# Kiripiro/leaffliction

Measured on AMD Instinct MI355X. Metric: 224x224 images/sec train, higher is better.
Workload: dtype f32; 1 GPU; leaf_cnn base train step (configs[1]: img 224, batch 256/GPU, fp32, 8 classes, AdamW+clipnorm+EMA, in-model augmentation); per_gpu_batch=256, global_batch=256, img_size=224, parallelism=dp1

## Files before the change

include/leafhip.h:

```cpp
#ifndef LEAFHIP_H
#define LEAFHIP_H

#include <stddef.h>
#include <stdint.h>

#ifdef __cplusplus
extern "C" {
#endif

#define LF_OK 0
#define LF_ERR_INVALID (-1)
#define LF_ERR_LAUNCH (-2)
#define LF_ERR_WORKSPACE (-3)

#define LF_VERSION 100

typedef void* lf_stream_t;

int lf_version(void);
const char* lf_last_error(void);

int lf_copy_rows(void* dst, size_t dst_pitch, const void* src, size_t src_pitch, size_t width, size_t rows, int to_host,
                 lf_stream_t stream);

// ... 122 lines not shown
                               const int32_t* ohw, const int64_t* out_off, int n, int h, int w,
                               int max_out_pixels, int fill, lf_stream_t stream);

int lf_resample_u8(const uint8_t* in, uint8_t* tmp, uint8_t* out, int n, int h, int w, int oh,
                   int ow, const int32_t* xbounds, const int32_t* xk, int kx,
                   const int32_t* ybounds, const int32_t* yk, int ky, int per_image_coeffs,
                   lf_stream_t stream);

int lf_resample_tile_u8(const uint8_t* in, uint8_t* out, int n, int h, int w, int oh, int ow,
                        const int32_t* xbounds, const int32_t* xk, int kx, const int32_t* ybounds,
                        const int32_t* yk, int ky, int per_image_coeffs, lf_stream_t stream);


int lf_conv2d_f32(const float* x, const float* w, float* y, int n, int cin, int h, int wd, int cout,
                  int ksize, const float* in_scale, const float* in_shift, int in_relu,
                  int accumulate, lf_stream_t stream);

size_t lf_conv2d_bf16_weight_elems(int cin, int cout, int ksize);
int lf_conv2d_bf16_prep_weights(const float* w_iko, uint16_t* wprep, int cin, int cout, int ksize,
                                lf_stream_t stream);
int lf_conv2d_bf16_f32(const float* x, const uint16_t* wprep, float* y, int n, int cin, int h, int wd,
                       int cout, int ksize, const float* in_scale, const float* in_shift, int in_relu,
                       lf_stream_t stream);

int lf_conv2d_bf16_act(const void* x, int x_bf16, const uint16_t* wprep, void* y, int y_bf16, int n,
                       int cin, int h, int wd, int cout, int ksize, const float* in_scale,
                       const float* in_shift, int in_relu, const float* out_scale,
                       const float* out_shift, int out_relu, lf_stream_t stream);
size_t lf_conv2d_bf16_act_mean_workspace(int n, int cin, int h, int wd, int cout, int ksize, int x_bf16);
int lf_conv2d_bf16_act_mean(const void* x, int x_bf16, const uint16_t* wprep, uint16_t* y, int n, int cin,
                            int h, int wd, int cout, int ksize, const float* in_scale,
// ... 32 lines not shown
int lf_cast_bf16_f32(const uint16_t* in, float* out, size_t count, lf_stream_t stream);

int lf_conv2d_variant(int h, int wd, int cout, int ksize);
int lf_conv2d_wgrad_variant(int n, int cin, int h, int wd, int cout, int ksize);

int lf_conv2d_plan(int n, int cin, int h, int wd, int cout, int ksize, int* out);
int lf_conv2d_wgrad_plan(int n, int cin, int h, int wd, int cout, int ksize, int* out);
int lf_conv2d_bf16_plan(int n, int cin, int h, int w, int cout, int ksize, int x_bf16, int y_bf16, int entry,
                        int accumulate, int mask, int* out);
int lf_conv2d_wgrad_bf16_plan(int n, int cin, int h, int w, int cout, int ksize, int* out);

long long lf_conv2d_stats_tiles(int n, int cin, int h, int w, int cout, int ksize);
int lf_conv2d_stats_f32(const float* x, const float* w, float* y, int n, int cin, int h, int wd,
                        int cout, int ksize, const float* in_scale, const float* in_shift,
                        int in_relu, const float* pivot, float* tile_part, size_t tile_part_bytes,
                        lf_stream_t stream);

int lf_conv2d_bnbwd_f32(const float* x, const float* w, float* y, int n, int cin, int h, int wd,
                        int cout, int ksize, int accumulate, const float* mask_y,
                        const float* mask_scale, const float* mask_shift, int mask_relu,
                        float* tile_part, size_t tile_part_bytes, lf_stream_t stream);

int lf_conv2d_dgrad_weights_f32(const float* w, float* wt, int cin, int ksize, int cout,
                                lf_stream_t stream);

size_t lf_conv2d_wgrad_workspace(int n, int cin, int h, int wd, int cout, int ksize);
int lf_conv2d_wgrad_f32(const float* x, const float* dy, int n, int cin, int h, int wd, int cout,
                        int ksize, const float* in_scale, const float* in_shift, int in_relu,
                        void* workspace, size_t ws_bytes, lf_stream_t stream);
int lf_conv2d_wgrad_reduce_f32(void* workspace, float* dw, int n, int cin, int h, int wd,
                               int cout, int ksize, float beta, lf_stream_t stream);
int lf_conv2d_wgrad_bn_supported(int n, int cin, int h, int w, int cout, int ksize);
int lf_conv2d_wgrad_bn_f32(const float* x, const float* g, const float* bn_y,
                           const float* alpha_nc, const float* add_nc, const float* coef,
                           int bn_relu, float* dy_out, int n, int cin, int h, int w, int cout,
                           int ksize, const float* in_scale, const float* in_shift, int in_relu,
                           void* workspace, size_t ws_bytes, lf_stream_t stream);

int lf_input_stage_f32(const uint8_t* in, float* out, int n, int h, int w, const float* aug4,
// ... 78 lines not shown
```

leaffliction_amd/_lib.py:

```python
from __future__ import annotations

import ctypes as C
import os
from pathlib import Path

_LIB = None

LIB_PATH = Path(__file__).resolve().parent / "libleafhip.so"

c_void_p, c_int, c_size_t, c_u64, c_float, c_double = (
    C.c_void_p, C.c_int, C.c_size_t, C.c_uint64, C.c_float, C.c_double)
P = c_void_p

SIGNATURES = {
    "lf_version": [],
    "lf_last_error": [],
    "lf_pack_hwc_u8_to_nchw_f32": [P, P, c_int, c_int, c_int, P, P, P],
    "lf_hist_u8": [P, P, c_int, c_int, c_int, P],
    "lf_autocontrast_lut": [P, P, P, c_int, P],
    "lf_lut_apply_u8": [P, P, P, c_int, c_int, c_int, P],
    "lf_gather_rows_u8": [P, P, P, c_int, c_size_t, P],
    "lf_flip_u8": [P, P, P, c_int, c_int, c_int, P],
    "lf_noise_wrap_add_u8": [P, P, P, c_size_t, P],
    "lf_add_wrap_u8": [P, P, P, c_size_t, P],
# ... 27 lines not shown
    "lf_inclusive_mask_u8": [P, P, c_int, c_int, c_int, c_int, c_int, P, P, c_size_t, P],
    "lf_make_mask_workspace": [c_int, c_int, c_int, c_int, c_int],
    "lf_make_mask_u8": [P, P, P, P, P, c_int, c_int, c_int, c_int, c_int, c_int, c_double, P, c_int, P, P,
                        c_size_t, P],
    "lf_brown_spots_workspace": [c_int, c_int, c_int],
    "lf_brown_spots_u8": [P, P, P, P, P, c_int, c_int, c_int, P, P, c_size_t, P],
    "lf_roi_u8": [P, P, P, c_int, P, P, P, P, c_int, c_int, c_int, c_int, c_int, P],
    "lf_blur_saliency_workspace": [c_int, c_int, c_int],
    "lf_blur_saliency_u8": [P, P, P, c_int, c_int, c_int, c_int, c_int, c_int, c_int, c_int, P, P, P,
                            c_size_t, P],
    "lf_warp_bicubic_u8": [P, P, P, c_int, c_int, c_int, c_int, P],
    "lf_affine_nearest_fixed_u8": [P, P, P, P, P, c_int, c_int, c_int, c_int, c_int, P],
    "lf_resample_tile_u8": [P, P, c_int, c_int, c_int, c_int, c_int, P, P, c_int, P, P, c_int, c_int, P],
    "lf_resample_u8": [P, P, P, c_int, c_int, c_int, c_int, c_int, P, P, c_int, P, P, c_int,
                       c_int, P],
    "lf_conv2d_f32": [P, P, P, c_int, c_int, c_int, c_int, c_int, c_int, P, P, c_int, c_int, P],
    "lf_conv2d_bf16_weight_elems": [c_int, c_int, c_int],
    "lf_conv2d_bf16_prep_weights": [P, P, c_int, c_int, c_int, P],
    "lf_conv2d_bf16_f32": [P, P, P, c_int, c_int, c_int, c_int, c_int, c_int, P, P, c_int, P],
    "lf_conv2d_bf16_act": [P, c_int, P, P, c_int, c_int, c_int, c_int, c_int, c_int, c_int, P, P, c_int,
                           P, P, c_int, P],
    "lf_conv2d_bf16_act_mean_workspace": [c_int, c_int, c_int, c_int, c_int, c_int, c_int],
    "lf_conv2d_bf16_act_mean": [P, c_int, P, P, c_int, c_int, c_int, c_int, c_int, c_int, P, P, c_int, P, P, c_int, P, P,
                                c_size_t, P],
    "lf_conv2d_bf16_stats_tiles": [c_int, c_int, c_int, c_int, c_int, c_int, c_int],
    "lf_conv2d_bf16_train": [P, c_int, P, P, c_int, c_int, c_int, c_int, c_int, c_int, P, P, c_int, c_int, P,
                             c_size_t, P, P, P, P, c_int, P],
    "lf_conv2d_wgrad_bf16_workspace": [c_int, c_int, c_int, c_int, c_int, c_int],
    "lf_conv2d_wgrad_bf16": [P, P, P, P, P, P, c_int, P, P, c_int, c_int, c_int, c_int, c_int, c_int, P, P,
                             c_int, P, c_size_t, P],
    "lf_gap_stats_bf16": [P, P, P, c_int, c_int, c_int, P, P, c_int, P],
    "lf_block_tail_fwd_train_bf16": [P, P, P, P, P, P, P, c_int, P, P, P, c_int, c_int, c_int, c_int, P],
    "lf_block_tail_bwd_bf16": [P, P, P, P, P, P, P, P, P, P, P, c_int, c_int, c_int, c_int, P],
    "lf_bcast_planes_bf16": [P, P, c_int, c_int, c_float, P],
    "lf_cast_f32_bf16": [P, P, c_size_t, P],
    "lf_cast_bf16_f32": [P, P, c_size_t, P],
    "lf_conv2d_variant": [c_int, c_int, c_int, c_int],
    "lf_conv2d_wgrad_variant": [c_int, c_int, c_int, c_int, c_int, c_int],
    "lf_conv2d_plan": [c_int, c_int, c_int, c_int, c_int, c_int, P],
    "lf_conv2d_wgrad_plan": [c_int, c_int, c_int, c_int, c_int, c_int, P],
    "lf_conv2d_bf16_plan": [c_int, c_int, c_int, c_int, c_int, c_int, c_int, c_int, c_int, c_int, c_int, P],
    "lf_conv2d_wgrad_bf16_plan": [c_int, c_int, c_int, c_int, c_int, c_int, P],
    "lf_conv2d_stats_tiles": [c_int, c_int, c_int, c_int, c_int, c_int],
    "lf_conv2d_stats_f32": [P, P, P, c_int, c_int, c_int, c_int, c_int, c_int, P, P, c_int, P, P, c_size_t, P],
    "lf_conv2d_bnbwd_f32": [P, P, P, c_int, c_int, c_int, c_int, c_int, c_int, c_int, P, P, P, c_int, P,
                            c_size_t, P],
    "lf_conv2d_dgrad_weights_f32": [P, P, c_int, c_int, c_int, P],
    "lf_conv2d_wgrad_workspace": [c_int, c_int, c_int, c_int, c_int, c_int],
    "lf_conv2d_wgrad_f32": [P, P, c_int, c_int, c_int, c_int, c_int, c_int, P, P, c_int, P,
                            c_size_t, P],
    "lf_conv2d_wgrad_bn_supported": [c_int, c_int, c_int, c_int, c_int, c_int],
    "lf_conv2d_wgrad_bn_f32": [P, P, P, P, P, P, c_int, P, c_int, c_int, c_int, c_int, c_int, c_int, P, P,
                               c_int, P, c_size_t, P],
    "lf_conv2d_wgrad_reduce_f32": [P, P, c_int, c_int, c_int, c_int, c_int, c_int, c_float, P],
    "lf_input_stage_f32": [P, P, c_int, c_int, c_int, P, P, P, P, P],
    "lf_scale_shift_act_f32": [P, P, c_int, c_int, c_int, P, P, c_int, P],
    "lf_bn_workspace": [c_int],
    "lf_bn_train_stats_f32": [P, c_int, c_int, c_int, P, P, P, P, c_float, c_float, P, P, P, P,
                              P, c_size_t, P],
    "lf_bn_train_stats_tiles_f32": [P, C.c_longlong, c_int, c_int, c_int, P, P, P, P, c_float, c_float, P, P, P, P, P, c_size_t, P],
    "lf_bn_bwd_sums_f32": [P, P, P, P, P, P, P, P, c_int, P, P, P, P, P, P, c_int, c_int, c_int, P,
                           c_size_t, P],
# ... 63 lines not shown
```

leaffliction_amd/csrc/lf_conv.hip:

```cpp
#include <type_traits>

#include "lf_common.h"

namespace {

typedef float f32x16 __attribute__((ext_vector_type(16)));
typedef float f32x4 __attribute__((ext_vector_type(4)));

constexpr int kThreads = 256;

__device__ __forceinline__ float pro_apply(float v, float sc, float sh, int relu) {
    v = fmaf(v, sc, sh);
    return relu ? fmaxf(v, 0.f) : v;
}

typedef float lf_f4 __attribute__((ext_vector_type(4)));
constexpr unsigned kBufOob = 0xffffffffu;
__device__ __forceinline__ __amdgpu_buffer_rsrc_t buf_rsrc(const float* base, unsigned bytes) {
    return __builtin_amdgcn_make_buffer_rsrc(const_cast<float*>(base), 0, bytes, 0x00020000);
}
__device__ __forceinline__ float4 buf_load4(__amdgpu_buffer_rsrc_t r, unsigned off) {
    const lf_f4 v = __builtin_bit_cast(lf_f4, __builtin_amdgcn_raw_buffer_load_b128(r, off, 0, 0));
    return make_float4(v.x, v.y, v.z, v.w);
}
__device__ __forceinline__ float buf_load1(__amdgpu_buffer_rsrc_t r, unsigned off) {
    return __builtin_bit_cast(float, __builtin_amdgcn_raw_buffer_load_b32(r, off, 0, 0));
}

struct ConvArgs {
    const float* x;
    const float* w;
    float* y;
    const float* in_scale;
    const float* in_shift;
    int n, cin, cout, h, wd;
    int tiles_x, tiles_y;
    int in_relu;
    int accumulate;
    int vec_ok;
    int stack;
    float* stat_part;
    const float* stat_pivot;
    long long stat_tiles;
    const float* stat_mask_y;
    const float* mask_scale;
    const float* mask_shift;
// ... 523 lines not shown
                    d[r * 4 + 0] = lo.x;
                    d[r * 4 + 1] = lo.y;
                    d[r * 4 + 2] = hi.x;
                    d[r * 4 + 3] = hi.y;
                }
                wino_input(d, v);
#pragma unroll
                for (int m = 0; m < MB; ++m)
#pragma unroll
                    for (int q = 0; q < 16; ++q)
                        wacc[m][nb][q] = __builtin_amdgcn_mfma_f32_16x16x4f32(u[m][q], v[q], wacc[m][nb][q], 0, 0, 0);
            }
        }
    };

    static_assert(kKC * CT <= kThreads, "one (channel, cout) filter per thread");
    const int ukc = tid / CT, uco = tid - ukc * CT;
    const bool u_on = tid < kKC * CT;
    const unsigned ugo = (u_on && co0 + uco < p.cout) ? 4u * ((unsigned)ukc * 9u * (unsigned)p.cout + (unsigned)(co0 + uco)) : kBufOob;
    float wr[9];
    auto load_u = [&](int c0) {
        const __amdgpu_buffer_rsrc_t rw =
            buf_rsrc(p.w + (size_t)c0 * 9 * p.cout, 4u * (unsigned)(min(kKC, p.cin - c0) * 9) * (unsigned)p.cout);
#pragma unroll
        for (int tap = 0; tap < 9; ++tap)
            wr[tap] = buf_load1(rw, ugo == kBufOob ? kBufOob : ugo + 4u * (unsigned)tap * (unsigned)p.cout);
    };
    auto store_u = [&]() {
        if (u_on) {
            float u[16];
            wino_filter(wr, u);
            float4* dst = reinterpret_cast<float4*>(lw + (ukc * CT + uco) * kUP);
#pragma unroll
            for (int q4 = 0; q4 < 4; ++q4) dst[q4] = make_float4(u[4 * q4], u[4 * q4 + 1], u[4 * q4 + 2], u[4 * q4 + 3]);
        }
    };

    const int nchunks = (p.cin + kKC - 1) / kKC;
    const bool vec = p.vec_ok && (t.tx0 + TW <= p.wd);

    if (vec) {
        constexpr bool kPrefetchW = NB == 1;
        Patch patch(p, t, lsc, tid);
        auto store_chunk = [&](int c0) {
            if (!kPrefetchW) load_u(c0);
            patch.store(p, lp, lsc, c0, tid);
            store_u();
        };
        patch.load(p, xin, 0);
        if (kPrefetchW) load_u(0);
        for (int ch = 0; ch < nchunks; ++ch) {
            __syncthreads();
            store_chunk(ch * kKC);
            __syncthreads();
            if (ch + 1 < nchunks) {
                patch.load(p, xin, (ch + 1) * kKC);
                if (kPrefetchW) load_u((ch + 1) * kKC);
            }
            compute_chunk();
        }
    } else {
        for (int ch = 0; ch < nchunks; ++ch) {
            const int c0 = ch * kKC;
            __syncthreads();
            Patch::stage_scalar(p, lp, xin, t.tx0, t.ty0, c0, tid);
            load_u(c0);
            store_u();
            __syncthreads();
            compute_chunk();
        }
    }

    float* yout = p.y + (size_t)t.n * p.cout * hw;
// ... 923 lines not shown
        float* o = dst + (size_t)g * count + i;
        *o = (final_pass && beta != 0.f) ? fmaf(beta, *o, s) : s;
    }
}

__global__ __launch_bounds__(kThreads) void weight_dgrad_kernel(const float* __restrict__ w,
                                                                float* __restrict__ wt, int cin,
                                                                int taps, int cout) {
    const int total = cin * taps * cout;
    for (int i = blockIdx.x * kThreads + threadIdx.x; i < total; i += gridDim.x * kThreads) {
        const int ci = i % cin, t = (i / cin) % taps, co = i / (cin * taps);
        wt[i] = w[((size_t)ci * taps + (taps - 1 - t)) * cout + co];
    }
}

struct FwdVariant {
    int tw, th, ct;
};
constexpr FwdVariant kFwdVariants[] = {{32, 8, 32}, {32, 8, 64}, {16, 16, 32}, {16, 16, 64},
                                       {28, 8, 128}, {32, 8, 128}, {56, 8, 64}};
constexpr int kNumFwd = sizeof(kFwdVariants) / sizeof(kFwdVariants[0]);

inline long long padded_work(const FwdVariant& v, int h, int w, int cout) {
    const long long tx = (w + v.tw - 1) / v.tw, ty = (h + v.th - 1) / v.th,
                    tc = (cout + v.ct - 1) / v.ct;
    return tx * v.tw * ty * v.th * tc * v.ct;
}

inline bool fwd_small_cin(int taps, int variant, int cin) { return taps == 9 && variant == 0 && cin <= 4; }

// ... 174 lines not shown
    return LF_OK;
}

int lf_conv2d_wgrad_plan(int n, int cin, int h, int wd, int cout, int ksize, int* out) {
    LF_REQUIRE(out, "lf_conv2d_wgrad_plan: null out");
    LF_REQUIRE(n > 0 && cin > 0 && cout > 0 && h > 0 && wd > 0 && (ksize == 1 || ksize == 3),
               "lf_conv2d_wgrad_plan: bad dims");
    const WgPlan pl = plan_wgrad(n, cin, cout, h, wd, ksize);
    out[0] = pl.variant;
    out[1] = pl.items_per_split < 3 ? pl.items_per_split : 3;
    out[2] = lf::slab_stages(pl.splits);
    out[3] = lf_conv2d_wgrad_bn_supported(n, cin, h, wd, cout, ksize);
    return LF_OK;
}

static int conv2d_launch(const char* who, const float* x, const float* w, float* y, int n, int cin,
                         int h, int wd, int cout, int ksize, const float* in_scale,
                         const float* in_shift, int in_relu, int accumulate, float* stat_part,
                         const float* stat_pivot, const float* stat_mask_y, const float* mask_scale,
                         const float* mask_shift, int mask_relu, lf_stream_t stream) {
    LF_REQUIRE(x && w && y, "%s: null buffer", who);
    LF_REQUIRE(n > 0 && cin > 0 && cout > 0 && h > 0 && wd > 0,
               "%s: bad dims n=%d cin=%d cout=%d h=%d w=%d", who, n, cin, cout, h, wd);
    LF_REQUIRE(ksize == 3 || ksize == 1, "%s: ksize must be 1 or 3 (got %d)", who, ksize);
    LF_REQUIRE((in_scale == nullptr) == (in_shift == nullptr),
               "%s: in_scale/in_shift must both be set", who);
    LF_REQUIRE(n <= 65535, "%s: batch too large for grid.z", who);
    LF_REQUIRE((size_t)cin * h * wd < (1ull << 30) && (size_t)cin * ksize * ksize * cout < (1ull << 30),
               "%s: per-image tensor too large for 32-bit offsets", who);
    const int best = lf_conv2d_variant(h, wd, cout, ksize);
    const FwdVariant& v = kFwdVariants[best];
    ConvArgs a;
    a.x = x; a.w = w; a.y = y; a.in_scale = in_scale; a.in_shift = in_shift;
    a.n = n; a.cin = cin; a.cout = cout; a.h = h; a.wd = wd;
    a.in_relu = in_relu;
    a.accumulate = accumulate;
    a.vec_ok = fwd_vec_shape(wd, cout) && aligned16(x) && aligned16(w);
    a.stack = conv_stack(best, n, cin, h, wd, cout);
    if (a.stack > 1 && !a.vec_ok) {
        if (stat_part != nullptr) {
            lf::set_error("%s: the statistics epilogue needs 16-byte aligned x / w", who);
            return LF_ERR_INVALID;
        }
        a.stack = 1;
    }
    a.tiles_x = (wd + v.tw - 1) / v.tw;
    a.tiles_y = (a.stack * h + v.th - 1) / v.th;
    a.stat_part = stat_part;
    a.stat_pivot = stat_pivot;
    a.stat_mask_y = stat_mask_y; a.mask_scale = mask_scale; a.mask_shift = mask_shift;
    a.mask_relu = mask_relu;
    const int gz = (n + a.stack - 1) / a.stack;
    a.stat_tiles = (long long)gz * a.tiles_x * a.tiles_y;
    const int rc = launch_fwd(ksize, best, a, a.tiles_x * a.tiles_y, gz, lf::as_stream(stream));
    if (rc != LF_OK) return rc;
    return lf::check_launch(who);
}

int lf_conv2d_f32(const float* x, const float* w, float* y, int n, int cin, int h, int wd, int cout,
                  int ksize, const float* in_scale, const float* in_shift, int in_relu,
                  int accumulate, lf_stream_t stream) {
    return conv2d_launch("lf_conv2d", x, w, y, n, cin, h, wd, cout, ksize, in_scale, in_shift, in_relu,
                         accumulate, nullptr, nullptr, nullptr, nullptr, nullptr, 0, stream);
}

long long lf_conv2d_stats_tiles(int n, int cin, int h, int wd, int cout, int ksize) {
    if (n <= 0 || cin <= 0 || h <= 0 || wd <= 0 || cout <= 0) return 0;
    const int best = lf_conv2d_variant(h, wd, cout, ksize);
    const FwdVariant& v = kFwdVariants[best];
    const int stack = conv_stack(best, n, cin, h, wd, cout);
    return (long long)((n + stack - 1) / stack) * ((wd + v.tw - 1) / v.tw) * ((stack * h + v.th - 1) / v.th);
}

int lf_conv2d_stats_f32(const float* x, const float* w, float* y, int n, int cin, int h, int wd,
                        int cout, int ksize, const float* in_scale, const float* in_shift,
                        int in_relu, const float* pivot, float* tile_part, size_t tile_part_bytes,
                        lf_stream_t stream) {
    LF_REQUIRE(tile_part, "lf_conv2d_stats: null tile_part");
    const long long tiles = lf_conv2d_stats_tiles(n, cin, h, wd, cout, ksize);
    if (tile_part_bytes < (size_t)tiles * (size_t)(cout > 0 ? cout : 0) * 2 * sizeof(float)) {
        lf::set_error("lf_conv2d_stats: tile_part %zu bytes < %lld tiles x %d channels x 8",
                      tile_part_bytes, tiles, cout);
        return LF_ERR_WORKSPACE;
    }
    return conv2d_launch("lf_conv2d_stats", x, w, y, n, cin, h, wd, cout, ksize, in_scale, in_shift,
                         in_relu, 0, tile_part, pivot, nullptr, nullptr, nullptr, 0, stream);
}

int lf_conv2d_bnbwd_f32(const float* x, const float* w, float* y, int n, int cin, int h, int wd,
                        int cout, int ksize, int accumulate, const float* mask_y,
                        const float* mask_scale, const float* mask_shift, int mask_relu,
                        float* tile_part, size_t tile_part_bytes, lf_stream_t stream) {
    LF_REQUIRE(tile_part && mask_y && mask_scale && mask_shift, "lf_conv2d_bnbwd: null buffer");
    const long long tiles = lf_conv2d_stats_tiles(n, cin, h, wd, cout, ksize);
    if (tile_part_bytes < (size_t)tiles * (size_t)(cout > 0 ? cout : 0) * 2 * sizeof(float)) {
        lf::set_error("lf_conv2d_bnbwd: tile_part %zu bytes < %lld tiles x %d channels x 8",
                      tile_part_bytes, tiles, cout);
        return LF_ERR_WORKSPACE;
    }
    return conv2d_launch("lf_conv2d_bnbwd", x, w, y, n, cin, h, wd, cout, ksize, nullptr, nullptr, 0,
                         accumulate, tile_part, nullptr, mask_y, mask_scale, mask_shift, mask_relu,
                         stream);
}

int lf_conv2d_dgrad_weights_f32(const float* w, float* wt, int cin, int ksize, int cout,
                                lf_stream_t stream) {
    LF_REQUIRE(w && wt, "lf_conv2d_dgrad_weights: null buffer");
    LF_REQUIRE(cin > 0 && cout > 0 && (ksize == 1 || ksize == 3), "lf_conv2d_dgrad_weights: bad dims");
    const int total = cin * ksize * ksize * cout;
    weight_dgrad_kernel<<<lf::stream_grid(total, kThreads), kThreads, 0, lf::as_stream(stream)>>>(
        w, wt, cin, ksize * ksize, cout);
    return lf::check_launch("lf_conv2d_dgrad_weights");
}

size_t lf_conv2d_wgrad_workspace(int n, int cin, int h, int wd, int cout, int ksize) {
    if (n <= 0 || cin <= 0 || cout <= 0 || h <= 0 || wd <= 0) return 0;
    const WgPlan pl = plan_wgrad(n, cin, cout, h, wd, ksize);
    const size_t count = (size_t)cin * ksize * ksize * cout;
    return ((size_t)pl.splits + lf::slab_groups(pl.splits)) * count * sizeof(float);
}

static int wgrad_launch(const char* who, const float* x, const float* dy, int n, int cin, int h,
                        int wd, int cout, int ksize, const float* in_scale, const float* in_shift,
                        int in_relu, const float* bn_y, const float* bn_alpha, const float* bn_add,
                        const float* bn_coef, int bn_relu, float* dy_out, void* workspace,
                        size_t ws_bytes, lf_stream_t stream) {
    LF_REQUIRE(x && dy && workspace, "%s: null buffer", who);
// ... 80 lines not shown
```

leaffliction_amd/model/cnn.py:

```python
from __future__ import annotations

import json
import os
import math
import zipfile
from pathlib import Path
from typing import Any, Dict, List, Optional, Tuple

import numpy as np
import torch

from .. import nn, ops

BN_MOMENTUM = 0.99
BN_EPS = 1e-3
NORM_EPS = 1e-7


def _specs(num_classes: int, widths: List[int], use_se: bool):
    out = [("stem.w", (3, 9, widths[0]), "w3"), ("stem.bn.gamma", (widths[0],), "vec"),
           ("stem.bn.beta", (widths[0],), "vec")]
    cin = widths[0]
    for i, f in enumerate(widths):
        p = f"s{i}."
# ... 261 lines not shown
        sc = torch.tensor([1.0 / d for d in denom], dtype=torch.float32, device=self.device)
        sh = torch.tensor([-m / d for m, d in zip(mean, denom)], dtype=torch.float32,
                          device=self.device)
        return nn.scale_shift_act(xc, sc, sh, False, out=out)

    def _bn(self, name: str, y: torch.Tensor, training: bool) -> torch.Tensor:
        st = self.stats[name]
        if training:
            nn.bn_train_stats(y, self.p[name + ".gamma"], self.p[name + ".beta"],
                              self.s[name + ".mean"], self.s[name + ".var"], st, BN_MOMENTUM, BN_EPS)
        else:
            nn.bn_infer_scale_shift(self.p[name + ".gamma"], self.p[name + ".beta"],
                                    self.s[name + ".mean"], self.s[name + ".var"], st, BN_EPS)
        return st

    def _conv_bn(self, x, wname: str, ksize: int, bn: str, pro, out: torch.Tensor, training: bool,
                 bf16: bool = False):
        P = self.p
        if training:
            st = self.stats[bn]
            bn_args = (P[bn + ".gamma"], P[bn + ".beta"], self.s[bn + ".mean"], self.s[bn + ".var"], st,
                       pro[0], pro[1], pro[2])
            if bf16:
                nn.conv2d_bn_stats_bf16(x, self._wt["f:" + wname], P[wname].shape[2], ksize, *bn_args,
                                        out=out, momentum=BN_MOMENTUM, eps=BN_EPS)
            else:
                nn.conv2d_bn_stats(x, P[wname], ksize, *bn_args, out=out, momentum=BN_MOMENTUM, eps=BN_EPS)
            return out, st
        w = P[wname]
        if self.infer_dtype == "bf16" and x.shape[3] % 4 == 0 and w.shape[2] % 32 == 0:
            y = nn.conv2d_bf16(x, nn.conv2d_bf16_weights(w, ksize), w.shape[2], ksize, pro[0], pro[1],
                               pro[2], out=out)
        else:
            y = nn.conv2d(x, w, ksize, pro[0], pro[1], pro[2], out=out)
        return y, self._bn(bn, y, False)

    def _bf16_storage_ok(self, h: int, w: int) -> bool:
        for f in self.widths:
            if f % 32 or w % 4 or h % 2:
                return False
            h, w = h // 2, w // 2
        return (h * w) % 4 == 0

    def _forward_infer_bf16(self, x0: torch.Tensor) -> torch.Tensor:
        n, _c, _h, _w = x0.shape
        P, bf = self.p, torch.bfloat16

        key = (self.flat_p._version, self.flat_s._version, self._mut)
        if self._infer_cache.get("key") != key:
# ... 200 lines not shown
            sv["bwd_dp"] = dp
            return
        bn_bwd_wgrad(sv["x0"], dp, sv["stem.y"], self.stats["stem.bn"], P["stem.bn.gamma"],
                     G["stem.bn.gamma"], G["stem.bn.beta"], True, 3, G["stem.w"], None,
                     tile_sums=stem_sums)

    def _dgrad(self, gy: torch.Tensor, wname: str, k: int, out: torch.Tensor, bf16: bool,
               accumulate: bool = False, mask=None):
        if bf16:
            wt, cin = self._wt["d:" + wname], self.p[wname].shape[0]
            if mask is None:
                nn.conv2d_bf16_train(gy, wt, cin, k, out, accumulate=accumulate)
                return None
            return nn.conv2d_bf16_train(gy, wt, cin, k, out, accumulate=accumulate, mask_y=mask[0],
                                        mask_scale=mask[1][2], mask_shift=mask[1][3], mask_relu=True)[1]
        wt = nn.conv2d_dgrad_weights(self.p[wname], k)
        if mask is None:
            nn.conv2d(gy, wt, k, out=out, accumulate=accumulate)
            return None
        return nn.conv2d_bnbwd(gy, wt, k, mask[0], mask[1], True, out, accumulate=accumulate)[1]

    def draw_dropout(self, n: int):
        host = []
        if self.drop_block > 0:
            host += [torch.empty((n, f)) for f in self.widths]
        if self.drop_top > 0:
            host.append(torch.empty((n, self.widths[-1])))
        self._host_dropout(n, host)
        drops = [t.to(self.device) for t in host[:len(self.widths)]] if self.drop_block > 0 else None
        top = host[-1].to(self.device) if self.drop_top > 0 else None
        return drops, top

    def train_step(self, x, y_true: Optional[torch.Tensor], lr: float, *, weight_decay: float = 1e-4,
                   clipnorm: float = 0.5, ema_decay: float = 0.999, adamw: bool = True,
                   grad_sync=None, global_n: Optional[int] = None, grad_overlap=None):
# ... 407 lines not shown
```

leaffliction_amd/nn.py:

```python
from __future__ import annotations

import os
from typing import Optional

import torch

from . import _lib
from .ops import _chk, _stream

_F32 = torch.float32
_ws_cache = {}
_ws_gen = 0
_NO_FUSED_BN_WGRAD = os.environ.get("LEAFFLICTION_NO_FUSED_BN_WGRAD", "0") == "1"


def _workspace(nbytes: int, device, slot: int = 0) -> torch.Tensor:
    global _ws_gen
    key = (str(device), slot)
    buf = _ws_cache.get(key)
    if buf is None or buf.numel() < nbytes:
        if torch.cuda.is_available() and torch.cuda.is_current_stream_capturing():
            raise RuntimeError("a workspace would have to grow while a HIP graph is being recorded: run the shape "
                               "eagerly first (the warm-up steps size every workspace)")
        buf = torch.empty(max(nbytes, 1 << 20), dtype=torch.uint8, device=device)
        _ws_cache[key] = buf
        _ws_gen += 1
    return buf


def workspace_generation() -> int:
    return _ws_gen


def _ptr(t: Optional[torch.Tensor]):
    return None if t is None else t.data_ptr()


def conv2d(x: torch.Tensor, w_iko: torch.Tensor, ksize: int, in_scale=None, in_shift=None,
           in_relu: bool = False, out: Optional[torch.Tensor] = None,
           accumulate: bool = False) -> torch.Tensor:
    _chk(x, _F32, "conv2d.x", 4)
    _chk(w_iko, _F32, "conv2d.w", 3)
    n, cin, h, w = x.shape
    if w_iko.shape[0] != cin or w_iko.shape[1] != ksize * ksize:
        raise ValueError(f"conv2d.w: expected [{cin},{ksize * ksize},Cout], got {tuple(w_iko.shape)}")
    cout = w_iko.shape[2]
    for t, nm in ((in_scale, "in_scale"), (in_shift, "in_shift")):
        if t is not None:
            _chk(t, _F32, f"conv2d.{nm}", 1)
            if t.shape[0] != cin:
                raise ValueError(f"conv2d.{nm}: expected [{cin}]")
    if out is None:
        if accumulate:
            raise ValueError("conv2d: accumulate needs an output tensor")
        out = torch.empty((n, cout, h, w), dtype=_F32, device=x.device)
    else:
        _chk(out, _F32, "conv2d.out", 4)
        if tuple(out.shape) != (n, cout, h, w):
            raise ValueError("conv2d.out: shape mismatch")
    _lib.call("lf_conv2d_f32", x.data_ptr(), w_iko.data_ptr(), out.data_ptr(), n, cin, h, w, cout,
              ksize, _ptr(in_scale), _ptr(in_shift), 1 if in_relu else 0, 1 if accumulate else 0,
              _stream())
    return out


def conv2d_bf16_weights(w_iko: torch.Tensor, ksize: int) -> torch.Tensor:
    _chk(w_iko, _F32, "conv2d_bf16_weights.w", 3)
    cin, taps, cout = w_iko.shape
    if taps != ksize * ksize:
        raise ValueError(f"conv2d_bf16_weights.w: expected [{cin},{ksize * ksize},Cout]")
    n = int(_lib.load().lf_conv2d_bf16_weight_elems(cin, cout, ksize))
    out = torch.empty(n, dtype=torch.int16, device=w_iko.device)
    _lib.call("lf_conv2d_bf16_prep_weights", w_iko.data_ptr(), out.data_ptr(), cin, cout, ksize, _stream())
    return out


def conv2d_bf16(x: torch.Tensor, wprep: torch.Tensor, cout: int, ksize: int, in_scale=None, in_shift=None,
# ... 161 lines not shown
              out.data_ptr(), n, cin, h, w, cout, ksize, _ptr(in_scale), _ptr(in_shift),
              1 if in_relu else 0, ws.data_ptr(), ws.numel(), _stream())
    return out


def cast_f32_bf16(src: torch.Tensor, dst: torch.Tensor) -> torch.Tensor:
    _lib.call("lf_cast_f32_bf16", src.data_ptr(), dst.data_ptr(), src.numel(), _stream())
    return dst


def cast_bf16_f32(src: torch.Tensor, dst: torch.Tensor) -> torch.Tensor:
    _lib.call("lf_cast_bf16_f32", src.data_ptr(), dst.data_ptr(), src.numel(), _stream())
    return dst


def conv2d_bn_stats(x: torch.Tensor, w_iko: torch.Tensor, ksize: int, gamma, beta, mmean, mvar,
                    stats: torch.Tensor, in_scale=None, in_shift=None, in_relu: bool = False,
                    out: Optional[torch.Tensor] = None, momentum: float = 0.99,
                    eps: float = 1e-3) -> torch.Tensor:
    _chk(x, _F32, "conv2d_bn_stats.x", 4)
    _chk(w_iko, _F32, "conv2d_bn_stats.w", 3)
    n, cin, h, w = x.shape
    if w_iko.shape[0] != cin or w_iko.shape[1] != ksize * ksize:
        raise ValueError(f"conv2d_bn_stats.w: expected [{cin},{ksize * ksize},Cout]")
    cout = w_iko.shape[2]
    for t, nm in ((in_scale, "in_scale"), (in_shift, "in_shift")):
        if t is not None:
            _chk(t, _F32, f"conv2d_bn_stats.{nm}", 1)
            if t.shape[0] != cin:
                raise ValueError(f"conv2d_bn_stats.{nm}: expected [{cin}]")
    for t in (gamma, beta, mmean, mvar):
        _chk(t, _F32, "conv2d_bn_stats.param", 1)
        if t.shape[0] != cout:
            raise ValueError("conv2d_bn_stats: per-channel vectors must be [Cout]")
    _chk(stats, _F32, "conv2d_bn_stats.stats", 2)
    if tuple(stats.shape) != (4, cout):
        raise ValueError("conv2d_bn_stats.stats: expected [4,Cout]")
    if out is None:
        out = torch.empty((n, cout, h, w), dtype=_F32, device=x.device)
    else:
        _chk(out, _F32, "conv2d_bn_stats.out", 4)
        if tuple(out.shape) != (n, cout, h, w):
            raise ValueError("conv2d_bn_stats.out: shape mismatch")
    lib = _lib.load()
    tiles = lib.lf_conv2d_stats_tiles(n, cin, h, w, cout, ksize)
    tp = _workspace(tiles * cout * 8, x.device, slot=1)
    _lib.call("lf_conv2d_stats_f32", x.data_ptr(), w_iko.data_ptr(), out.data_ptr(), n, cin, h, w,
              cout, ksize, _ptr(in_scale), _ptr(in_shift), 1 if in_relu else 0, mmean.data_ptr(),
              tp.data_ptr(), tp.numel(), _stream())
    ws = _workspace(lib.lf_bn_workspace(cout), x.device)
    _lib.call("lf_bn_train_stats_tiles_f32", tp.data_ptr(), tiles, n, cout, h * w, gamma.data_ptr(),
              beta.data_ptr(), mmean.data_ptr(), mvar.data_ptr(), float(momentum), float(eps),
              stats[0].data_ptr(), stats[1].data_ptr(), stats[2].data_ptr(), stats[3].data_ptr(),
              ws.data_ptr(), ws.numel(), _stream())
    return out


def conv2d_bnbwd(x: torch.Tensor, w_iko: torch.Tensor, ksize: int, mask_y: torch.Tensor,
                 stats: torch.Tensor, relu: bool, out: torch.Tensor, accumulate: bool = False):
    _chk(x, _F32, "conv2d_bnbwd.x", 4)
    _chk(w_iko, _F32, "conv2d_bnbwd.w", 3)
    _chk(mask_y, _F32, "conv2d_bnbwd.mask_y", 4)
    _chk(out, _F32, "conv2d_bnbwd.out", 4)
    n, cin, h, w = x.shape
    if w_iko.shape[0] != cin or w_iko.shape[1] != ksize * ksize:
        raise ValueError(f"conv2d_bnbwd.w: expected [{cin},{ksize * ksize},Cout]")
    cout = w_iko.shape[2]
    if tuple(out.shape) != (n, cout, h, w) or mask_y.shape != out.shape or tuple(stats.shape) != (4, cout):
        raise ValueError("conv2d_bnbwd: shape mismatch")
    tiles = _lib.load().lf_conv2d_stats_tiles(n, cin, h, w, cout, ksize)
    tp = _workspace(tiles * cout * 8, x.device, slot=1)
    _lib.call("lf_conv2d_bnbwd_f32", x.data_ptr(), w_iko.data_ptr(), out.data_ptr(), n, cin, h, w,
              cout, ksize, 1 if accumulate else 0, mask_y.data_ptr(), stats[2].data_ptr(),
              stats[3].data_ptr(), 1 if relu else 0, tp.data_ptr(), tp.numel(), _stream())
    return out, (tp, tiles)


def conv2d_dgrad_weights(w_iko: torch.Tensor, ksize: int) -> torch.Tensor:
    _chk(w_iko, _F32, "dgrad_weights.w", 3)
    cin, taps, cout = w_iko.shape
    if taps != ksize * ksize:
        raise ValueError("dgrad_weights: taps != ksize^2")
    wt = torch.empty((cout, taps, cin), dtype=_F32, device=w_iko.device)
    _lib.call("lf_conv2d_dgrad_weights_f32", w_iko.data_ptr(), wt.data_ptr(), cin, ksize, cout,
              _stream())
    return wt


def conv2d_wgrad(x: torch.Tensor, dy: torch.Tensor, ksize: int, in_scale=None, in_shift=None,
# ... 308 lines not shown
```

Baseline: 5913 images/sec.

## Precompute Winograd filter transforms once per step instead of per tile

Adds a kernel that transforms 3x3 weights into 4x4 Winograd-domain filters, with a flipped and transposed variant for dgrad, and stores them in a per-weight buffer. The forward and bnbwd conv kernels now load the pretransformed filters as float4 instead of loading 9 taps and running the filter transform in every block for every channel chunk. This also removes the separate dgrad weight-transpose launch on Winograd paths. In exchange it adds a transform launch per conv and per direction, plus 16/9 more weight bytes read per chunk, and it drops the weight prefetch overlap.

```diff
diff --git a/include/leafhip.h b/include/leafhip.h
--- a/include/leafhip.h
+++ b/include/leafhip.h
@@ -160,7 +160,7 @@
 
 int lf_conv2d_f32(const float* x, const float* w, float* y, int n, int cin, int h, int wd, int cout,
                   int ksize, const float* in_scale, const float* in_shift, int in_relu,
-                  int accumulate, lf_stream_t stream);
+                  int accumulate, lf_stream_t stream, const float* wino_u);
 
 size_t lf_conv2d_bf16_weight_elems(int cin, int cout, int ksize);
 int lf_conv2d_bf16_prep_weights(const float* w_iko, uint16_t* wprep, int cin, int cout, int ksize,
@@ -223,15 +223,18 @@
 int lf_conv2d_stats_f32(const float* x, const float* w, float* y, int n, int cin, int h, int wd,
                         int cout, int ksize, const float* in_scale, const float* in_shift,
                         int in_relu, const float* pivot, float* tile_part, size_t tile_part_bytes,
-                        lf_stream_t stream);
+                        lf_stream_t stream, const float* wino_u);
 
 int lf_conv2d_bnbwd_f32(const float* x, const float* w, float* y, int n, int cin, int h, int wd,
                         int cout, int ksize, int accumulate, const float* mask_y,
                         const float* mask_scale, const float* mask_shift, int mask_relu,
-                        float* tile_part, size_t tile_part_bytes, lf_stream_t stream);
+                        float* tile_part, size_t tile_part_bytes, lf_stream_t stream, const float* wino_u);
 
 int lf_conv2d_dgrad_weights_f32(const float* w, float* wt, int cin, int ksize, int cout,
                                 lf_stream_t stream);
+
+int lf_conv2d_takes_wino_filters(int cin, int h, int wd, int cout, int ksize);
+int lf_conv2d_wino_filters_f32(const float* w, float* u, int cin, int cout, int dgrad, lf_stream_t stream);
 
 size_t lf_conv2d_wgrad_workspace(int n, int cin, int h, int wd, int cout, int ksize);
 int lf_conv2d_wgrad_f32(const float* x, const float* dy, int n, int cin, int h, int wd, int cout,
diff --git a/leaffliction_amd/_lib.py b/leaffliction_amd/_lib.py
--- a/leaffliction_amd/_lib.py
+++ b/leaffliction_amd/_lib.py
@@ -65,7 +65,7 @@
     "lf_resample_tile_u8": [P, P, c_int, c_int, c_int, c_int, c_int, P, P, c_int, P, P, c_int, c_int, P],
     "lf_resample_u8": [P, P, P, c_int, c_int, c_int, c_int, c_int, P, P, c_int, P, P, c_int,
                        c_int, P],
-    "lf_conv2d_f32": [P, P, P, c_int, c_int, c_int, c_int, c_int, c_int, P, P, c_int, c_int, P],
+    "lf_conv2d_f32": [P, P, P, c_int, c_int, c_int, c_int, c_int, c_int, P, P, c_int, c_int, P, P],
     "lf_conv2d_bf16_weight_elems": [c_int, c_int, c_int],
     "lf_conv2d_bf16_prep_weights": [P, P, c_int, c_int, c_int, P],
     "lf_conv2d_bf16_f32": [P, P, P, c_int, c_int, c_int, c_int, c_int, c_int, P, P, c_int, P],
@@ -93,10 +93,12 @@
     "lf_conv2d_bf16_plan": [c_int, c_int, c_int, c_int, c_int, c_int, c_int, c_int, c_int, c_int, c_int, P],
     "lf_conv2d_wgrad_bf16_plan": [c_int, c_int, c_int, c_int, c_int, c_int, P],
     "lf_conv2d_stats_tiles": [c_int, c_int, c_int, c_int, c_int, c_int],
-    "lf_conv2d_stats_f32": [P, P, P, c_int, c_int, c_int, c_int, c_int, c_int, P, P, c_int, P, P, c_size_t, P],
+    "lf_conv2d_stats_f32": [P, P, P, c_int, c_int, c_int, c_int, c_int, c_int, P, P, c_int, P, P, c_size_t, P, P],
     "lf_conv2d_bnbwd_f32": [P, P, P, c_int, c_int, c_int, c_int, c_int, c_int, c_int, P, P, P, c_int, P,
-                            c_size_t, P],
+                            c_size_t, P, P],
     "lf_conv2d_dgrad_weights_f32": [P, P, c_int, c_int, c_int, P],
+    "lf_conv2d_takes_wino_filters": [c_int, c_int, c_int, c_int, c_int],
+    "lf_conv2d_wino_filters_f32": [P, P, c_int, c_int, c_int, P],
     "lf_conv2d_wgrad_workspace": [c_int, c_int, c_int, c_int, c_int, c_int],
     "lf_conv2d_wgrad_f32": [P, P, c_int, c_int, c_int, c_int, c_int, c_int, P, P, c_int, P,
                             c_size_t, P],
diff --git a/leaffliction_amd/csrc/lf_conv.hip b/leaffliction_amd/csrc/lf_conv.hip
--- a/leaffliction_amd/csrc/lf_conv.hip
+++ b/leaffliction_amd/csrc/lf_conv.hip
@@ -30,6 +30,7 @@
 struct ConvArgs {
     const float* x;
     const float* w;
+    const float* wino_u;
     float* y;
     const float* in_scale;
     const float* in_shift;
@@ -583,49 +584,37 @@
         }
     };
 
-    static_assert(kKC * CT <= kThreads, "one (channel, cout) filter per thread");
-    const int ukc = tid / CT, uco = tid - ukc * CT;
-    const bool u_on = tid < kKC * CT;
-    const unsigned ugo = (u_on && co0 + uco < p.cout) ? 4u * ((unsigned)ukc * 9u * (unsigned)p.cout + (unsigned)(co0 + uco)) : kBufOob;
-    float wr[9];
+    constexpr int KSTEP = kThreads / (4 * CT), UPT = kKC / KSTEP;
+    static_assert(kThreads % (4 * CT) == 0 && kKC % KSTEP == 0, "whole channels per pass");
+    const int ukc = tid / (4 * CT), uco = (tid >> 2) % CT, uq4 = tid & 3;
+    const unsigned ustep = 64u * KSTEP * (unsigned)p.cout;
+    const unsigned ugo = co0 + uco < p.cout ? 4u * (((unsigned)ukc * (unsigned)p.cout + (unsigned)(co0 + uco)) * 16u + 4u * (unsigned)uq4) : 0x80000000u;
+    float* const ulds = lw + (ukc * CT + uco) * kUP + 4 * uq4;
+    float4 uv[UPT];
     auto load_u = [&](int c0) {
-        const __amdgpu_buffer_rsrc_t rw =
-            buf_rsrc(p.w + (size_t)c0 * 9 * p.cout, 4u * (unsigned)(min(kKC, p.cin - c0) * 9) * (unsigned)p.cout);
-#pragma unroll
-        for (int tap = 0; tap < 9; ++tap)
-            wr[tap] = buf_load1(rw, ugo == kBufOob ? kBufOob : ugo + 4u * (unsigned)tap * (unsigned)p.cout);
+        const __amdgpu_buffer_rsrc_t ru =
+            buf_rsrc(p.wino_u + (size_t)c0 * p.cout * 16, 64u * (unsigned)min(kKC, p.cin - c0) * (unsigned)p.cout);
+#pragma unroll
+        for (int i = 0; i < UPT; ++i) uv[i] = buf_load4(ru, ugo + (unsigned)i * ustep);
     };
     auto store_u = [&]() {
-        if (u_on) {
-            float u[16];
-            wino_filter(wr, u);
-            float4* dst = reinterpret_cast<float4*>(lw + (ukc * CT + uco) * kUP);
-#pragma unroll
-            for (int q4 = 0; q4 < 4; ++q4) dst[q4] = make_float4(u[4 * q4], u[4 * q4 + 1], u[4 * q4 + 2], u[4 * q4 + 3]);
-        }
+#pragma unroll
+        for (int i = 0; i < UPT; ++i) *reinterpret_cast<float4*>(ulds + i * KSTEP * CT * kUP) = uv[i];
     };
 
     const int nchunks = (p.cin + kKC - 1) / kKC;
     const bool vec = p.vec_ok && (t.tx0 + TW <= p.wd);
 
     if (vec) {
-        constexpr bool kPrefetchW = NB == 1;
         Patch patch(p, t, lsc, tid);
-        auto store_chunk = [&](int c0) {
-            if (!kPrefetchW) load_u(c0);
-            patch.store(p, lp, lsc, c0, tid);
-            store_u();
-        };
         patch.load(p, xin, 0);
-        if (kPrefetchW) load_u(0);
         for (int ch = 0; ch < nchunks; ++ch) {
             __syncthreads();
-            store_chunk(ch * kKC);
+            load_u(ch * kKC);
+            patch.store(p, lp, lsc, ch * kKC, tid);
+            store_u();
             __syncthreads();
-            if (ch + 1 < nchunks) {
-                patch.load(p, xin, (ch + 1) * kKC);
-                if (kPrefetchW) load_u((ch + 1) * kKC);
-            }
+            if (ch + 1 < nchunks) patch.load(p, xin, (ch + 1) * kKC);
             compute_chunk();
         }
     } else {
@@ -1579,6 +1568,22 @@
     }
 }
 
+__global__ __launch_bounds__(kThreads) void wino_filters_kernel(const float* __restrict__ w,
+                                                                float* __restrict__ u, int cin, int cout,
+                                                                int dgrad) {
+    const int total = cin * cout;
+    for (int i = blockIdx.x * kThreads + threadIdx.x; i < total; i += gridDim.x * kThreads) {
+        const int ci = i / cout, co = i - ci * cout;
+        float g[9], t[16];
+#pragma unroll
+        for (int tap = 0; tap < 9; ++tap) g[tap] = w[((size_t)ci * 9 + (dgrad ? 8 - tap : tap)) * cout + co];
+        wino_filter(g, t);
+        float4* dst = reinterpret_cast<float4*>(u + (dgrad ? (size_t)co * cin + ci : (size_t)i) * 16);
+#pragma unroll
+        for (int q4 = 0; q4 < 4; ++q4) dst[q4] = make_float4(t[4 * q4], t[4 * q4 + 1], t[4 * q4 + 2], t[4 * q4 + 3]);
+    }
+}
+
 struct FwdVariant {
     int tw, th, ct;
 };
@@ -1783,12 +1788,16 @@
     return LF_OK;
 }
 
-static int conv2d_launch(const char* who, const float* x, const float* w, float* y, int n, int cin,
+static inline bool fwd_takes_wino_filters(int cin, int h, int wd, int cout, int ksize) {
+    return ksize == 3 && !fwd_small_cin(9, lf_conv2d_variant(h, wd, cout, ksize), cin);
+}
+
+static int conv2d_launch(const char* who, const float* x, const float* w, const float* wino_u, float* y, int n, int cin,
                          int h, int wd, int cout, int ksize, const float* in_scale,
                          const float* in_shift, int in_relu, int accumulate, float* stat_part,
                          const float* stat_pivot, const float* stat_mask_y, const float* mask_scale,
                          const float* mask_shift, int mask_relu, lf_stream_t stream) {
-    LF_REQUIRE(x && w && y, "%s: null buffer", who);
+    LF_REQUIRE(x && y, "%s: null buffer", who);
     LF_REQUIRE(n > 0 && cin > 0 && cout > 0 && h > 0 && wd > 0,
                "%s: bad dims n=%d cin=%d cout=%d h=%d w=%d", who, n, cin, cout, h, wd);
     LF_REQUIRE(ksize == 3 || ksize == 1, "%s: ksize must be 1 or 3 (got %d)", who, ksize);
@@ -1799,12 +1808,22 @@
                "%s: per-image tensor too large for 32-bit offsets", who);
     const int best = lf_conv2d_variant(h, wd, cout, ksize);
     const FwdVariant& v = kFwdVariants[best];
+    if (fwd_takes_wino_filters(cin, h, wd, cout, ksize)) {
+        LF_REQUIRE(wino_u, "%s: this 3x3 convolution runs in the Winograd domain and needs wino_u "
+                   "(lf_conv2d_wino_filters_f32)", who);
+        LF_REQUIRE(aligned16(wino_u), "%s: wino_u must be 16-byte aligned", who);
+        LF_REQUIRE((size_t)cin * cout * 16 < (1ull << 30) && cout <= (1 << 20), "%s: wino_u too large for 32-bit offsets", who);
+    } else {
+        LF_REQUIRE(w, "%s: null buffer", who);
+    }
     ConvArgs a;
-    a.x = x; a.w = w; a.y = y; a.in_scale = in_scale; a.in_shift = in_shift;
+    a.x = x; a.w = w; a.y = y;
+    a.wino_u = fwd_takes_wino_filters(cin, h, wd, cout, ksize) ? wino_u : nullptr;
+    a.in_scale = in_scale; a.in_shift = in_shift;
     a.n = n; a.cin = cin; a.cout = cout; a.h = h; a.wd = wd;
     a.in_relu = in_relu;
     a.accumulate = accumulate;
-    a.vec_ok = fwd_vec_shape(wd, cout) && aligned16(x) && aligned16(w);
+    a.vec_ok = fwd_vec_shape(wd, cout) && aligned16(x) && aligned16(a.wino_u ? nullptr : w);
     a.stack = conv_stack(best, n, cin, h, wd, cout);
     if (a.stack > 1 && !a.vec_ok) {
         if (stat_part != nullptr) {
@@ -1828,8 +1847,8 @@
 
 int lf_conv2d_f32(const float* x, const float* w, float* y, int n, int cin, int h, int wd, int cout,
                   int ksize, const float* in_scale, const float* in_shift, int in_relu,
-                  int accumulate, lf_stream_t stream) {
-    return conv2d_launch("lf_conv2d", x, w, y, n, cin, h, wd, cout, ksize, in_scale, in_shift, in_relu,
+                  int accumulate, lf_stream_t stream, const float* wino_u) {
+    return conv2d_launch("lf_conv2d", x, w, wino_u, y, n, cin, h, wd, cout, ksize, in_scale, in_shift, in_relu,
                          accumulate, nullptr, nullptr, nullptr, nullptr, nullptr, 0, stream);
 }
 
@@ -1844,7 +1863,7 @@
 int lf_conv2d_stats_f32(const float* x, const float* w, float* y, int n, int cin, int h, int wd,
                         int cout, int ksize, const float* in_scale, const float* in_shift,
                         int in_relu, const float* pivot, float* tile_part, size_t tile_part_bytes,
-                        lf_stream_t stream) {
+                        lf_stream_t stream, const float* wino_u) {
     LF_REQUIRE(tile_part, "lf_conv2d_stats: null tile_part");
     const long long tiles = lf_conv2d_stats_tiles(n, cin, h, wd, cout, ksize);
     if (tile_part_bytes < (size_t)tiles * (size_t)(cout > 0 ? cout : 0) * 2 * sizeof(float)) {
@@ -1852,14 +1871,14 @@
                       tile_part_bytes, tiles, cout);
         return LF_ERR_WORKSPACE;
     }
-    return conv2d_launch("lf_conv2d_stats", x, w, y, n, cin, h, wd, cout, ksize, in_scale, in_shift,
+    return conv2d_launch("lf_conv2d_stats", x, w, wino_u, y, n, cin, h, wd, cout, ksize, in_scale, in_shift,
                          in_relu, 0, tile_part, pivot, nullptr, nullptr, nullptr, 0, stream);
 }
 
 int lf_conv2d_bnbwd_f32(const float* x, const float* w, float* y, int n, int cin, int h, int wd,
                         int cout, int ksize, int accumulate, const float* mask_y,
                         const float* mask_scale, const float* mask_shift, int mask_relu,
-                        float* tile_part, size_t tile_part_bytes, lf_stream_t stream) {
+                        float* tile_part, size_t tile_part_bytes, lf_stream_t stream, const float* wino_u) {
     LF_REQUIRE(tile_part && mask_y && mask_scale && mask_shift, "lf_conv2d_bnbwd: null buffer");
     const long long tiles = lf_conv2d_stats_tiles(n, cin, h, wd, cout, ksize);
     if (tile_part_bytes < (size_t)tiles * (size_t)(cout > 0 ? cout : 0) * 2 * sizeof(float)) {
@@ -1867,7 +1886,7 @@
                       tile_part_bytes, tiles, cout);
         return LF_ERR_WORKSPACE;
     }
-    return conv2d_launch("lf_conv2d_bnbwd", x, w, y, n, cin, h, wd, cout, ksize, nullptr, nullptr, 0,
+    return conv2d_launch("lf_conv2d_bnbwd", x, w, wino_u, y, n, cin, h, wd, cout, ksize, nullptr, nullptr, 0,
                          accumulate, tile_part, nullptr, mask_y, mask_scale, mask_shift, mask_relu,
                          stream);
 }
@@ -1880,6 +1899,20 @@
     weight_dgrad_kernel<<<lf::stream_grid(total, kThreads), kThreads, 0, lf::as_stream(stream)>>>(
         w, wt, cin, ksize * ksize, cout);
     return lf::check_launch("lf_conv2d_dgrad_weights");
+}
+
+int lf_conv2d_takes_wino_filters(int cin, int h, int wd, int cout, int ksize) {
+    if (cin <= 0 || cout <= 0 || h <= 0 || wd <= 0) return 0;
+    return fwd_takes_wino_filters(cin, h, wd, cout, ksize) ? 1 : 0;
+}
+
+int lf_conv2d_wino_filters_f32(const float* w, float* u, int cin, int cout, int dgrad, lf_stream_t stream) {
+    LF_REQUIRE(w && u, "lf_conv2d_wino_filters: null buffer");
+    LF_REQUIRE(cin > 0 && cout > 0 && (size_t)cin * cout * 16 < (1ull << 30), "lf_conv2d_wino_filters: bad dims");
+    LF_REQUIRE(aligned16(u), "lf_conv2d_wino_filters: u must be 16-byte aligned");
+    wino_filters_kernel<<<lf::stream_grid((size_t)cin * cout, kThreads), kThreads, 0, lf::as_stream(stream)>>>(
+        w, u, cin, cout, dgrad ? 1 : 0);
+    return lf::check_launch("lf_conv2d_wino_filters");
 }
 
 size_t lf_conv2d_wgrad_workspace(int n, int cin, int h, int wd, int cout, int ksize) {
diff --git a/leaffliction_amd/model/cnn.py b/leaffliction_amd/model/cnn.py
--- a/leaffliction_amd/model/cnn.py
+++ b/leaffliction_amd/model/cnn.py
@@ -299,6 +299,15 @@
                                     self.s[name + ".mean"], self.s[name + ".var"], st, BN_EPS)
         return st
 
+    def _wino_u(self, wname: str, ksize: int, hw, dgrad: bool = False) -> Optional[torch.Tensor]:
+        cin, _taps, cout = self.p[wname].shape
+        if dgrad:
+            cin, cout = cout, cin
+        if not nn.conv2d_takes_wino_filters(cin, hw[0], hw[1], cout, ksize):
+            return None
+        u = self._buf("wino", ("d:" if dgrad else "f:") + wname, (cin, cout, 16))
+        return nn.conv2d_wino_filters(self.p[wname], dgrad, out=u)
+
     def _conv_bn(self, x, wname: str, ksize: int, bn: str, pro, out: torch.Tensor, training: bool,
                  bf16: bool = False):
         P = self.p
@@ -310,14 +319,16 @@
                 nn.conv2d_bn_stats_bf16(x, self._wt["f:" + wname], P[wname].shape[2], ksize, *bn_args,
                                         out=out, momentum=BN_MOMENTUM, eps=BN_EPS)
             else:
-                nn.conv2d_bn_stats(x, P[wname], ksize, *bn_args, out=out, momentum=BN_MOMENTUM, eps=BN_EPS)
+                nn.conv2d_bn_stats(x, P[wname], ksize, *bn_args, out=out, momentum=BN_MOMENTUM, eps=BN_EPS,
+                                   wino_u=self._wino_u(wname, ksize, x.shape[2:]))
             return out, st
         w = P[wname]
         if self.infer_dtype == "bf16" and x.shape[3] % 4 == 0 and w.shape[2] % 32 == 0:
             y = nn.conv2d_bf16(x, nn.conv2d_bf16_weights(w, ksize), w.shape[2], ksize, pro[0], pro[1],
                                pro[2], out=out)
         else:
-            y = nn.conv2d(x, w, ksize, pro[0], pro[1], pro[2], out=out)
+            y = nn.conv2d(x, w, ksize, pro[0], pro[1], pro[2], out=out,
+                          wino_u=self._wino_u(wname, ksize, x.shape[2:]))
         return y, self._bn(bn, y, False)
 
     def _bf16_storage_ok(self, h: int, w: int) -> bool:
@@ -548,11 +559,12 @@
                 return None
             return nn.conv2d_bf16_train(gy, wt, cin, k, out, accumulate=accumulate, mask_y=mask[0],
                                         mask_scale=mask[1][2], mask_shift=mask[1][3], mask_relu=True)[1]
-        wt = nn.conv2d_dgrad_weights(self.p[wname], k)
+        u = self._wino_u(wname, k, gy.shape[2:], dgrad=True)
+        wt = nn.conv2d_dgrad_weights(self.p[wname], k) if u is None else None
         if mask is None:
-            nn.conv2d(gy, wt, k, out=out, accumulate=accumulate)
+            nn.conv2d(gy, wt, k, out=out, accumulate=accumulate, wino_u=u)
             return None
-        return nn.conv2d_bnbwd(gy, wt, k, mask[0], mask[1], True, out, accumulate=accumulate)[1]
+        return nn.conv2d_bnbwd(gy, wt, k, mask[0], mask[1], True, out, accumulate=accumulate, wino_u=u)[1]
 
     def draw_dropout(self, n: int):
         host = []
diff --git a/leaffliction_amd/nn.py b/leaffliction_amd/nn.py
--- a/leaffliction_amd/nn.py
+++ b/leaffliction_amd/nn.py
@@ -36,15 +36,60 @@
     return None if t is None else t.data_ptr()
 
 
-def conv2d(x: torch.Tensor, w_iko: torch.Tensor, ksize: int, in_scale=None, in_shift=None,
+def conv2d_takes_wino_filters(cin: int, h: int, w: int, cout: int, ksize: int) -> bool:
+    return bool(_lib.load().lf_conv2d_takes_wino_filters(int(cin), int(h), int(w), int(cout), int(ksize)))
+
+
+def conv2d_wino_filters(w_iko: torch.Tensor, dgrad: bool = False,
+                        out: Optional[torch.Tensor] = None) -> torch.Tensor:
+    _chk(w_iko, _F32, "conv2d_wino_filters.w", 3)
+    cin, taps, cout = w_iko.shape
+    if taps != 9:
+        raise ValueError("conv2d_wino_filters: 3x3 weights [Cin,9,Cout] expected")
+    shape = (cout, cin, 16) if dgrad else (cin, cout, 16)
+    if out is None:
+        out = torch.empty(shape, dtype=_F32, device=w_iko.device)
+    else:
+        _chk(out, _F32, "conv2d_wino_filters.out", 3)
+        if tuple(out.shape) != shape:
+            raise ValueError(f"conv2d_wino_filters.out: expected {shape}")
+    _lib.call("lf_conv2d_wino_filters_f32", w_iko.data_ptr(), out.data_ptr(), cin, cout, 1 if dgrad else 0,
+              _stream())
+    return out
+
+
+def _conv_weights(who: str, x: torch.Tensor, w_iko: Optional[torch.Tensor], ksize: int,
+                  wino_u: Optional[torch.Tensor]):
+    n, cin, h, w = x.shape
+    if w_iko is not None:
+        _chk(w_iko, _F32, f"{who}.w", 3)
+        if w_iko.shape[0] != cin or w_iko.shape[1] != ksize * ksize:
+            raise ValueError(f"{who}.w: expected [{cin},{ksize * ksize},Cout], got {tuple(w_iko.shape)}")
+        cout = w_iko.shape[2]
+    elif wino_u is not None:
+        cout = wino_u.shape[1] if wino_u.dim() == 3 else 0
+    else:
+        raise ValueError(f"{who}: no weights")
+    if not conv2d_takes_wino_filters(cin, h, w, cout, ksize):
+        if w_iko is None:
+            raise ValueError(f"{who}: this launch reads the raw weights, not wino_u")
+        return cout, w_iko.data_ptr(), None
+    if wino_u is None:
+        ws = _workspace(cin * cout * 64, x.device, slot=3)
+        wino_u = conv2d_wino_filters(w_iko, out=ws[:cin * cout * 64].view(_F32).view(cin, cout, 16))
+    else:
+        _chk(wino_u, _F32, f"{who}.wino_u", 3)
+        if tuple(wino_u.shape) != (cin, cout, 16):
+            raise ValueError(f"{who}.wino_u: expected [{cin},{cout},16], got {tuple(wino_u.shape)}")
+    return cout, _ptr(w_iko), wino_u.data_ptr()
+
+
+def conv2d(x: torch.Tensor, w_iko: Optional[torch.Tensor], ksize: int, in_scale=None, in_shift=None,
            in_relu: bool = False, out: Optional[torch.Tensor] = None,
-           accumulate: bool = False) -> torch.Tensor:
+           accumulate: bool = False, wino_u: Optional[torch.Tensor] = None) -> torch.Tensor:
     _chk(x, _F32, "conv2d.x", 4)
-    _chk(w_iko, _F32, "conv2d.w", 3)
-    n, cin, h, w = x.shape
-    if w_iko.shape[0] != cin or w_iko.shape[1] != ksize * ksize:
-        raise ValueError(f"conv2d.w: expected [{cin},{ksize * ksize},Cout], got {tuple(w_iko.shape)}")
-    cout = w_iko.shape[2]
+    n, cin, h, w = x.shape
+    cout, w_ptr, u_ptr = _conv_weights("conv2d", x, w_iko, ksize, wino_u)
     for t, nm in ((in_scale, "in_scale"), (in_shift, "in_shift")):
         if t is not None:
             _chk(t, _F32, f"conv2d.{nm}", 1)
@@ -58,9 +103,9 @@
         _chk(out, _F32, "conv2d.out", 4)
         if tuple(out.shape) != (n, cout, h, w):
             raise ValueError("conv2d.out: shape mismatch")
-    _lib.call("lf_conv2d_f32", x.data_ptr(), w_iko.data_ptr(), out.data_ptr(), n, cin, h, w, cout,
+    _lib.call("lf_conv2d_f32", x.data_ptr(), w_ptr, out.data_ptr(), n, cin, h, w, cout,
               ksize, _ptr(in_scale), _ptr(in_shift), 1 if in_relu else 0, 1 if accumulate else 0,
-              _stream())
+              _stream(), u_ptr)
     return out
 
 
@@ -252,16 +297,13 @@
     return dst
 
 
-def conv2d_bn_stats(x: torch.Tensor, w_iko: torch.Tensor, ksize: int, gamma, beta, mmean, mvar,
+def conv2d_bn_stats(x: torch.Tensor, w_iko: Optional[torch.Tensor], ksize: int, gamma, beta, mmean, mvar,
                     stats: torch.Tensor, in_scale=None, in_shift=None, in_relu: bool = False,
                     out: Optional[torch.Tensor] = None, momentum: float = 0.99,
-                    eps: float = 1e-3) -> torch.Tensor:
+                    eps: float = 1e-3, wino_u: Optional[torch.Tensor] = None) -> torch.Tensor:
     _chk(x, _F32, "conv2d_bn_stats.x", 4)
-    _chk(w_iko, _F32, "conv2d_bn_stats.w", 3)
-    n, cin, h, w = x.shape
-    if w_iko.shape[0] != cin or w_iko.shape[1] != ksize * ksize:
-        raise ValueError(f"conv2d_bn_stats.w: expected [{cin},{ksize * ksize},Cout]")
-    cout = w_iko.shape[2]
+    n, cin, h, w = x.shape
+    cout, w_ptr, u_ptr = _conv_weights("conv2d_bn_stats", x, w_iko, ksize, wino_u)
     for t, nm in ((in_scale, "in_scale"), (in_shift, "in_shift")):
         if t is not None:
             _chk(t, _F32, f"conv2d_bn_stats.{nm}", 1)
@@ -283,9 +325,9 @@
     lib = _lib.load()
     tiles = lib.lf_conv2d_stats_tiles(n, cin, h, w, cout, ksize)
     tp = _workspace(tiles * cout * 8, x.device, slot=1)
-    _lib.call("lf_conv2d_stats_f32", x.data_ptr(), w_iko.data_ptr(), out.data_ptr(), n, cin, h, w,
+    _lib.call("lf_conv2d_stats_f32", x.data_ptr(), w_ptr, out.data_ptr(), n, cin, h, w,
               cout, ksize, _ptr(in_scale), _ptr(in_shift), 1 if in_relu else 0, mmean.data_ptr(),
-              tp.data_ptr(), tp.numel(), _stream())
+              tp.data_ptr(), tp.numel(), _stream(), u_ptr)
     ws = _workspace(lib.lf_bn_workspace(cout), x.device)
     _lib.call("lf_bn_train_stats_tiles_f32", tp.data_ptr(), tiles, n, cout, h * w, gamma.data_ptr(),
               beta.data_ptr(), mmean.data_ptr(), mvar.data_ptr(), float(momentum), float(eps),
@@ -294,23 +336,21 @@
     return out
 
 
-def conv2d_bnbwd(x: torch.Tensor, w_iko: torch.Tensor, ksize: int, mask_y: torch.Tensor,
-                 stats: torch.Tensor, relu: bool, out: torch.Tensor, accumulate: bool = False):
+def conv2d_bnbwd(x: torch.Tensor, w_iko: Optional[torch.Tensor], ksize: int, mask_y: torch.Tensor,
+                 stats: torch.Tensor, relu: bool, out: torch.Tensor, accumulate: bool = False,
+                 wino_u: Optional[torch.Tensor] = None):
     _chk(x, _F32, "conv2d_bnbwd.x", 4)
-    _chk(w_iko, _F32, "conv2d_bnbwd.w", 3)
     _chk(mask_y, _F32, "conv2d_bnbwd.mask_y", 4)
     _chk(out, _F32, "conv2d_bnbwd.out", 4)
     n, cin, h, w = x.shape
-    if w_iko.shape[0] != cin or w_iko.shape[1] != ksize * ksize:
-        raise ValueError(f"conv2d_bnbwd.w: expected [{cin},{ksize * ksize},Cout]")
-    cout = w_iko.shape[2]
+    cout, w_ptr, u_ptr = _conv_weights("conv2d_bnbwd", x, w_iko, ksize, wino_u)
     if tuple(out.shape) != (n, cout, h, w) or mask_y.shape != out.shape or tuple(stats.shape) != (4, cout):
         raise ValueError("conv2d_bnbwd: shape mismatch")
     tiles = _lib.load().lf_conv2d_stats_tiles(n, cin, h, w, cout, ksize)
     tp = _workspace(tiles * cout * 8, x.device, slot=1)
-    _lib.call("lf_conv2d_bnbwd_f32", x.data_ptr(), w_iko.data_ptr(), out.data_ptr(), n, cin, h, w,
+    _lib.call("lf_conv2d_bnbwd_f32", x.data_ptr(), w_ptr, out.data_ptr(), n, cin, h, w,
               cout, ksize, 1 if accumulate else 0, mask_y.data_ptr(), stats[2].data_ptr(),
-              stats[3].data_ptr(), 1 if relu else 0, tp.data_ptr(), tp.numel(), _stream())
+              stats[3].data_ptr(), 1 if relu else 0, tp.data_ptr(), tp.numel(), _stream(), u_ptr)
     return out, (tp, tiles)
 
 
```

Measured after the change: 6164 images/sec, median of 6. +4.3%, better.
